# ForJadeForest/DistillCLIP

Measured on AMD Instinct MI355X. Metric: image-text pairs/sec (distill step), higher is better.
Workload: dtype bf16; 1 GPU; l_clip.yaml dual distill: ViT-B/32 CLIP teacher -> weight-shared ViT(6x768,24h,R2) + text(4x768,12h,R2) students, 224px/77tok, losses out_l1+out_cos+0.1*cos_diff, fwd+loss+bwd+AdamW; global_batch=512, batch_per_gpu=512, parallelism=dp1, gradient_exchange=none, negatives=local (reference training_step semantics), optimizer_in_step=True, teacher_residual=fp16, saved_gelu_derivative=u8 fixed point, clock_probe=True

## Files before the change

distillclip_amd/csrc/common.h:

```cpp
#pragma once
#include <hip/hip_runtime.h>
#include <stdint.h>

typedef __bf16 bf16_t;
typedef __attribute__((ext_vector_type(8))) __bf16 bf16x8;
typedef __attribute__((ext_vector_type(4))) __bf16 bf16x4;
typedef __attribute__((ext_vector_type(2))) __bf16 bf16x2;
typedef __attribute__((ext_vector_type(8))) _Float16 f16x8;
typedef __attribute__((ext_vector_type(4))) _Float16 f16x4;
typedef __attribute__((ext_vector_type(4))) short s16x4;
typedef __attribute__((ext_vector_type(4))) float f32x4;
typedef __attribute__((ext_vector_type(16))) float f32x16;
typedef __attribute__((ext_vector_type(4))) unsigned int u32x4;

#include "dclip.h"

void dclip_set_error(const char* fmt, ...);

#define DCLIP_REQUIRE(cond, ...)                 \
    do {                                          \
        if (!(cond)) {                            \
            dclip_set_error(__VA_ARGS__);         \
            return DCLIP_EINVAL;                  \
        }                                         \
    } while (0)

extern "C" int dclip_rows_pick(const void* src, void* dst, const int32_t* idx, int64_t B, int64_t row_bytes, void* stream);
extern "C" int dclip_rows_expand(const void* src, void* dst, const int32_t* idx, int64_t B, int64_t N, int64_t row_bytes, void* stream);

extern "C" int dclip_cast_bf16_pad(const float* src, void* dst, int64_t R, int64_t C, int64_t ldd, void* stream);

bool dclip_trace_open(int kind, double flops, double bytes, void* stream, int* slot, int d0 = 0, int d1 = 0, int d2 = 0, int d3 = 0);
void dclip_trace_close(int slot, void* stream);
struct TraceScope {
    int slot = -1; void* st;
    TraceScope(int kind, double flops, double bytes, void* stream, int d0 = 0, int d1 = 0, int d2 = 0, int d3 = 0) : st(stream) {
        if (!dclip_trace_open(kind, flops, bytes, stream, &slot, d0, d1, d2, d3)) slot = -1;
    }
    ~TraceScope() { if (slot >= 0) dclip_trace_close(slot, st); }
};
#define DCLIP_TRACE_GEMM_NT 0
#define DCLIP_TRACE_GEMM_TN 1
#define DCLIP_TRACE_LAYERNORM 2
#define DCLIP_TRACE_LOSS 3
#define DCLIP_TRACE_ATTN 4
#define DCLIP_TRACE_LN_BWD 5

void dclip_explain_hip_error(const char* what, int hip_error, const char* hip_text);
static inline int dclip_check_launch(const char* what) {
    hipError_t e = hipGetLastError();
    if (e != hipSuccess) {
        dclip_explain_hip_error(what, (int)e, hipGetErrorString(e));
        return DCLIP_ELAUNCH;
    }
    return DCLIP_OK;
}

static inline int grid_for(int64_t work, int per_block = 256, int cap = 2048 * 4) {
    int64_t g = (work + per_block - 1) / per_block;
    return (int)(g < 1 ? 1 : (g > cap ? cap : g));
}

static inline size_t dclip_up256(size_t x) { return (x + 255) & ~(size_t)255; }
static inline bool dclip_aligned16(const void* p) { return ((uintptr_t)p % 16) == 0; }
struct Bump {
    char* base; size_t off;
    explicit Bump(void* b) : base((char*)b), off(0) {}
    template <class T> T* take(size_t n) {
        T* p = base ? (T*)(base + off) : nullptr;
        off += dclip_up256(n * sizeof(T));
        return p;
    }
};

__device__ __forceinline__ float bf2f(bf16_t x) { return (float)x; }
__device__ __forceinline__ bf16_t f2bf(float x) { return (bf16_t)x; }

__device__ __forceinline__ float wave_sum(float v) {
#pragma unroll
    for (int o = 32; o > 0; o >>= 1) v += __shfl_xor(v, o);
    return v;
}
__device__ __forceinline__ float wave_max(float v) {
#pragma unroll
    for (int o = 32; o > 0; o >>= 1) v = fmaxf(v, __shfl_xor(v, o));
    return v;
}

__device__ __forceinline__ void wave_lds_fence() { __builtin_amdgcn_wave_barrier(); asm volatile("" ::: "memory"); __builtin_amdgcn_wave_barrier(); }

template <class T> __device__ __forceinline__ void mfma_keep_alive(const T& f) { asm volatile("" :: "v"(f)); }
template <class T> __device__ __forceinline__ void mfma_keep_alive(const T (&f)[2]) { asm volatile("" :: "v"(f[0]), "v"(f[1])); }
template <class T> __device__ __forceinline__ void mfma_keep_alive(const T (&f)[4]) { asm volatile("" :: "v"(f[0]), "v"(f[1]), "v"(f[2]), "v"(f[3])); }

__device__ __forceinline__ float quick_gelu_f(float x) { return x * __builtin_amdgcn_rcpf(1.f + __expf(-1.702f * x)); }
__device__ __forceinline__ float erf_tail(float ax_over_sqrt2, float phi) {
    const float t = __builtin_amdgcn_rcpf(fmaf(0.3275911f, ax_over_sqrt2, 1.f));
    float p = fmaf(1.061405429f, t, -1.453152027f);
    p = fmaf(p, t, 1.421413741f);
    p = fmaf(p, t, -0.284496736f);
    p = fmaf(p, t, 0.254829592f);
    return p * t * phi;
}
__device__ __forceinline__ float gelu_erf_f(float x) {
    const float phi = __expf(-0.5f * x * x);
    const float tail = erf_tail(fabsf(x) * 0.70710678118654752f, phi);
    const float cdf = x >= 0.f ? 1.f - 0.5f * tail : 0.5f * tail;
    return x * cdf;
}
__device__ __forceinline__ float dgelu_erf_f(float x) {
    const float phi = __expf(-0.5f * x * x);
    const float tail = erf_tail(fabsf(x) * 0.70710678118654752f, phi);
    const float cdf = x >= 0.f ? 1.f - 0.5f * tail : 0.5f * tail;
    return fmaf(x * phi, 0.3989422804014327f, cdf);
}

__device__ __forceinline__ void gelu_erf_both_f(float x, float& g, float& dg) {
    const float phi = __expf(-0.5f * x * x);
    const float tail = erf_tail(fabsf(x) * 0.70710678118654752f, phi);
    const float cdf = x >= 0.f ? 1.f - 0.5f * tail : 0.5f * tail;
    g = x * cdf;
    dg = fmaf(x * phi, 0.3989422804014327f, cdf);
}

#define DCLIP_DG_LO (-0.13f)
#define DCLIP_DG_STEP (1.26f / 255.f)
__device__ __forceinline__ unsigned dg_pack4(float a, float b, float c, float d) {
    const float inv = 255.f / 1.26f, off = 0.13f * (255.f / 1.26f);
    unsigned r = 0;
    r = __builtin_amdgcn_cvt_pk_u8_f32(__builtin_rintf(fmaf(a, inv, off)), 0, r);
    r = __builtin_amdgcn_cvt_pk_u8_f32(__builtin_rintf(fmaf(b, inv, off)), 1, r);
    r = __builtin_amdgcn_cvt_pk_u8_f32(__builtin_rintf(fmaf(c, inv, off)), 2, r);
    r = __builtin_amdgcn_cvt_pk_u8_f32(__builtin_rintf(fmaf(d, inv, off)), 3, r);
    return r;
}
__device__ __forceinline__ float dg_unpack(unsigned w, int byte) {
    return fmaf((float)((w >> (8 * byte)) & 0xffu), DCLIP_DG_STEP, DCLIP_DG_LO);
}

__device__ __forceinline__ bf16x8 frag_halves(s16x4 lo, s16x4 hi) {
    union { struct { s16x4 lo, hi; } s; bf16x8 v; } u;
    u.s.lo = lo; u.s.hi = hi;
    return u.v;
}

typedef __attribute__((address_space(3))) s16x4 lds_s16x4;
template <int ROWB>
__device__ __forceinline__ bf16x8 tr_frag(const char* tile, int r0, int x0, int lane) {
    const int g = lane >> 4, q = (lane >> 2) & 3, pp = lane & 3;
    const char* a0 = tile + (r0 + 8 * g + q) * ROWB + (x0 + 4 * pp) * 2;
    return frag_halves(__builtin_amdgcn_ds_read_tr16_b64_v4i16((lds_s16x4*)a0), __builtin_amdgcn_ds_read_tr16_b64_v4i16((lds_s16x4*)(a0 + 4 * ROWB)));
}

__device__ __forceinline__ int xcd_remap(int bid, int nwg) {
    const int q = nwg >> 3, r = nwg & 7, x = bid & 7;
    return (x < r ? x * (q + 1) : r * (q + 1) + (x - r) * q) + (bid >> 3);
}
```

distillclip_amd/csrc/gemm_common.h:

```cpp
#pragma once
#include <math.h>
#include <stdlib.h>
#include "common.h"
#include <type_traits>

namespace dgemm {

constexpr int BM = 128, BN = 128, BK = 64;
constexpr int SUB = 1024;
constexpr int HT = 16384;

inline unsigned long long* g_gemm_stamps = nullptr;

struct GemmNT {
    const bf16_t* A; int64_t lda;
    const bf16_t* B; int64_t ldb;
    void* C; int64_t ldc;
    int M, N, K;
    float alpha;
    const float* bias;
    const void* aux_in;
    void* aux_out;
    const void* residual; int64_t ldr;
    int row_group; const float* rowadd;
    float* colsum;
    int tiles_m, tiles_n;
    unsigned long long* stamps;
    int group_n;
    unsigned long long* clk;
};

__device__ __forceinline__ int swz(int x) { return x ^ (((x >> 9) & 1) << 5); }

typedef __attribute__((address_space(3))) void lds_void;
typedef __attribute__((address_space(1))) const void gbl_void;

struct EpiSide {
    float4 r0, r1;
    f16x8 rh;
    bf16x8 z;
    uint2 zq;
};

template <int ACT, int OUT>
__device__ __forceinline__ void epilogue_load_side(const GemmNT& p, int64_t o, int64_t orr, EpiSide& sd) {
    if (OUT == 1 && p.residual) {
        const float* rp = (const float*)p.residual + orr;
        sd.r0 = *(const float4*)rp; sd.r1 = *(const float4*)(rp + 4);
    }
    if (OUT == 2 && p.residual) sd.rh = *(const f16x8*)((const _Float16*)p.residual + orr);
    if (ACT == 3) sd.z = *(const bf16x8*)((const bf16_t*)p.aux_in + o);
    if (ACT == 4) sd.zq = *(const uint2*)((const uint8_t*)p.aux_in + o);
}

template <int ACT, int OUT, int MODE = 0, bool CSUM_ALWAYS = false>
__device__ __forceinline__ void epilogue_vec8(const GemmNT& p, float (&v)[8], int row, int col, int64_t o, int64_t orr,
                                              const float (&bias)[8], float (&csum)[8], const EpiSide& sd) {
    constexpr bool LEAN = MODE != 0;
#pragma unroll
    for (int e = 0; e < 8; ++e) v[e] = v[e] * p.alpha + bias[e];
    if (!LEAN && p.row_group > 0) {
        const float* ra = p.rowadd + (int64_t)(row % p.row_group) * p.N + col;
        const float4 a0 = *(const float4*)ra, a1 = *(const float4*)(ra + 4);
        v[0] += a0.x; v[1] += a0.y; v[2] += a0.z; v[3] += a0.w; v[4] += a1.x; v[5] += a1.y; v[6] += a1.z; v[7] += a1.w;
    }
    if (!LEAN && ACT != 5 && ACT != 6 && p.aux_out) {
        bf16x8 z;
#pragma unroll
        for (int e = 0; e < 8; ++e) z[e] = f2bf(v[e]);
        *(bf16x8*)((bf16_t*)p.aux_out + o) = z;
    }
    if (ACT == 1) {
#pragma unroll
        for (int e = 0; e < 8; ++e) v[e] = quick_gelu_f(v[e]);
    }
    if (ACT == 2) {
#pragma unroll
        for (int e = 0; e < 8; ++e) v[e] = gelu_erf_f(v[e]);
    }
    if (ACT == 3) {
        const bf16x8 z = sd.z;
#pragma unroll
        for (int e = 0; e < 8; ++e) v[e] *= dgelu_erf_f(bf2f(z[e]));
    }
    if (ACT == 4) {
        const uint2 q = sd.zq;
        v[0] *= dg_unpack(q.x, 0); v[1] *= dg_unpack(q.x, 1); v[2] *= dg_unpack(q.x, 2); v[3] *= dg_unpack(q.x, 3);
        v[4] *= dg_unpack(q.y, 0); v[5] *= dg_unpack(q.y, 1); v[6] *= dg_unpack(q.y, 2); v[7] *= dg_unpack(q.y, 3);
    }
    if (ACT == 5) {
        float dg[8];
#pragma unroll
        for (int e = 0; e < 8; ++e) {
            float g;
            gelu_erf_both_f(v[e], g, dg[e]);
            v[e] = g;
        }
        if (LEAN || p.aux_out) *(uint2*)((uint8_t*)p.aux_out + o) = uint2{dg_pack4(dg[0], dg[1], dg[2], dg[3]), dg_pack4(dg[4], dg[5], dg[6], dg[7])};
    }
    if (ACT == 6) {
        float dg[8];
#pragma unroll
        for (int e = 0; e < 8; ++e) {
            const float sg = __builtin_amdgcn_rcpf(1.f + __expf(-1.702f * v[e]));
            dg[e] = fmaf(1.702f * v[e] * sg, 1.f - sg, sg);
            v[e] *= sg;
        }
        if (LEAN || p.aux_out) *(uint2*)((uint8_t*)p.aux_out + o) = uint2{dg_pack4(dg[0], dg[1], dg[2], dg[3]), dg_pack4(dg[4], dg[5], dg[6], dg[7])};
    }
    if (MODE == 3 || (!LEAN && p.residual)) {
        if (OUT == 2) {
            const f16x8 r = sd.rh;
#pragma unroll
            for (int e = 0; e < 8; ++e) v[e] += (float)r[e];
        } else {
            float4 r0, r1;
            if (OUT == 1) { r0 = sd.r0; r1 = sd.r1; }
            else {
                const float* rp = (const float*)p.residual + orr;
                r0 = *(const float4*)rp; r1 = *(const float4*)(rp + 4);
            }
            v[0] += r0.x; v[1] += r0.y; v[2] += r0.z; v[3] += r0.w; v[4] += r1.x; v[5] += r1.y; v[6] += r1.z; v[7] += r1.w;
        }
    }
    if (OUT == 1) {
        float* cp = (float*)p.C + o;
        *(float4*)cp = float4{v[0], v[1], v[2], v[3]};
        *(float4*)(cp + 4) = float4{v[4], v[5], v[6], v[7]};
    } else if (OUT == 2) {
        f16x8 ov;
#pragma unroll
        for (int e = 0; e < 8; ++e) ov[e] = (_Float16)v[e];
        *(f16x8*)((_Float16*)p.C + o) = ov;
    } else {
        bf16x8 ov;
#pragma unroll
        for (int e = 0; e < 8; ++e) ov[e] = f2bf(v[e]);
        *(bf16x8*)((bf16_t*)p.C + o) = ov;
    }
    if (CSUM_ALWAYS || (OUT == 0 && (MODE == 2 || (MODE == 0 && p.colsum)))) {
#pragma unroll
        for (int e = 0; e < 8; ++e) csum[e] += v[e];
    }
}

#define WAIT_VMCNT(n) asm volatile("s_waitcnt vmcnt(" #n ")" ::: "memory")
#define WAIT_LGKM0() asm volatile("s_waitcnt lgkmcnt(0)" ::: "memory")

__device__ __forceinline__ void wg_stamp(unsigned long long* const& stamps, const int& tid, int k) {
    if (stamps && tid == 0) {
        if (k == 3) WAIT_VMCNT(0);
        stamps[6 * (int64_t)blockIdx.x + k] = __builtin_readcyclecounter();
        if (k == 0) stamps[6 * (int64_t)blockIdx.x + 4] = __builtin_amdgcn_s_memrealtime();
        if (k == 3) stamps[6 * (int64_t)blockIdx.x + 5] = __builtin_amdgcn_s_memrealtime();
    }
}

__device__ __forceinline__ void mfma_4x4(f32x4 (&acc)[4][4], const bf16x8 (&a)[4], const bf16x8 (&b)[4]) {
#pragma unroll
    for (int i = 0; i < 4; ++i)
#pragma unroll
        for (int j = 0; j < 4; ++j) acc[i][j] = __builtin_amdgcn_mfma_f32_16x16x32_bf16(a[i], b[j], acc[i][j], 0, 0, 0);
}

template <bool SWAP>
__device__ __forceinline__ f32x4 mfma_rc(bf16x8 rowf, bf16x8 colf, f32x4 c) {
    return SWAP ? __builtin_amdgcn_mfma_f32_16x16x32_bf16(colf, rowf, c, 0, 0, 0) : __builtin_amdgcn_mfma_f32_16x16x32_bf16(rowf, colf, c, 0, 0, 0);
}
#define PHASE_MFMA(SWAP, acc, R0, RT, af, b0, b1)                                                                         \
    do {                                                                                                                  \
        __builtin_amdgcn_s_barrier();                                                                                     \
        __builtin_amdgcn_s_setprio(1);                                                                                    \
        _Pragma("unroll") for (int kb_ = 0; kb_ < 2; ++kb_)                                                               \
            _Pragma("unroll") for (int i_ = 0; i_ < (RT); ++i_) {                                                         \
                _Pragma("unroll") for (int j_ = 0; j_ < 2; ++j_)                                                          \
                    acc[(R0) + i_][j_] = mfma_rc<SWAP>(af[i_][kb_], b0[j_][kb_], acc[(R0) + i_][j_]);                     \
                _Pragma("unroll") for (int j_ = 0; j_ < 2; ++j_)                                                          \
                    acc[(R0) + i_][2 + j_] = mfma_rc<SWAP>(af[i_][kb_], b1[j_][kb_], acc[(R0) + i_][2 + j_]);             \
            }                                                                                                             \
        __builtin_amdgcn_s_setprio(0);                                                                                    \
        __builtin_amdgcn_s_barrier();                                                                                     \
    } while (0)

template <int NI, int LD>
__device__ __forceinline__ void stage_acc(float* cs, const f32x4 (*acc)[4], int row0, int col0, int lane) {
#pragma unroll
    for (int i = 0; i < NI; ++i)
#pragma unroll
        for (int j = 0; j < 4; ++j)
#pragma unroll
            for (int r = 0; r < 4; ++r) cs[(row0 + i * 16 + (lane >> 4) * 4 + r) * LD + col0 + j * 16 + (lane & 15)] = acc[i][j][r];
}

}
```

distillclip_amd/csrc/gemm_nt.hip:

```cpp

#include "gemm_common.h"
#include <atomic>

using namespace dgemm;

namespace {

constexpr int TILE_BYTES = (BM / 16) * (BK / 32) * SUB;
constexpr int CLD = BN + 4;
constexpr int NT_LDS = (4 * TILE_BYTES > BM * CLD * 4) ? 4 * TILE_BYTES : BM * CLD * 4;


__device__ __forceinline__ void stage_operand(const bf16_t* __restrict__ G, int64_t ld, int row0, int rows_max,
                                              int k0, char* lds_tile, int wave, int lane) {
    const int L = lane * 16;
    const int X = swz(L);
    const int r = X >> 6, c = (X >> 4) & 3;
#pragma unroll
    for (int s = 0; s < 4; ++s) {
        const int sub = wave * 4 + s;
        const int rb = sub >> 1, kb = sub & 1;
        int row = row0 + rb * 16 + r;
        row = row < rows_max ? row : rows_max - 1;
        const bf16_t* src = G + (int64_t)row * ld + (k0 + kb * 32 + c * 8);
        __builtin_amdgcn_global_load_lds((gbl_void*)src, (lds_void*)(lds_tile + sub * SUB), 16, 0, 0);
    }
}

template <int ACT, int OUT>
__global__ __launch_bounds__(256) void gemm_nt_kernel(GemmNT p) {
    extern __shared__ __attribute__((aligned(16))) char smem[];
    const int tid = threadIdx.x, lane = tid & 63;
    const int wave = __builtin_amdgcn_readfirstlane(tid >> 6);
    const int wm = wave >> 1, wn = wave & 1;

    const int nwg = p.tiles_m * p.tiles_n;
    const int t = xcd_remap(blockIdx.x, nwg);
    const int tm = t / p.tiles_n, tn = t % p.tiles_n;
    const int m0 = tm * BM, n0 = tn * BN;

    char* As = smem;
    char* Bs = smem + 2 * TILE_BYTES;

    f32x4 acc[4][4];
#pragma unroll
    for (int i = 0; i < 4; ++i)
#pragma unroll
        for (int j = 0; j < 4; ++j) acc[i][j] = f32x4{0.f, 0.f, 0.f, 0.f};

    const int nk = p.K / BK;
    stage_operand(p.A, p.lda, m0, p.M, 0, As, wave, lane);
    stage_operand(p.B, p.ldb, n0, p.N, 0, Bs, wave, lane);

    const int fragoff = swz((lane & 15) * 64 + (lane >> 4) * 16);

    for (int kt = 0; kt < nk; ++kt) {
        __syncthreads();
        if (kt + 1 < nk) {
            const int nb = (kt + 1) & 1;
            stage_operand(p.A, p.lda, m0, p.M, (kt + 1) * BK, As + nb * TILE_BYTES, wave, lane);
            stage_operand(p.B, p.ldb, n0, p.N, (kt + 1) * BK, Bs + nb * TILE_BYTES, wave, lane);
        }
        const char* a_t = As + (kt & 1) * TILE_BYTES;
        const char* b_t = Bs + (kt & 1) * TILE_BYTES;
#pragma unroll
        for (int kb = 0; kb < 2; ++kb) {
            bf16x8 af[4], bfr[4];
#pragma unroll
            for (int i = 0; i < 4; ++i)
                af[i] = *(const bf16x8*)(a_t + ((wm * 4 + i) * 2 + kb) * SUB + fragoff);
#pragma unroll
            for (int j = 0; j < 4; ++j)
                bfr[j] = *(const bf16x8*)(b_t + ((wn * 4 + j) * 2 + kb) * SUB + fragoff);
            mfma_4x4(acc, af, bfr);
        }
    }

    __syncthreads();
    float* cs = (float*)smem;
    stage_acc<4, CLD>(cs, acc, wm * 64, wn * 64, lane);
    __syncthreads();
    const int cc = (tid & 15) * 8;
    const int col = n0 + cc;
    const bool col_ok = col < p.N;
    float bias[8], csum[8];
#pragma unroll
    for (int e = 0; e < 8; ++e) { bias[e] = 0.f; csum[e] = 0.f; }
    if (p.bias && col_ok) {
        const float4 b0 = *(const float4*)(p.bias + col), b1 = *(const float4*)(p.bias + col + 4);
        bias[0] = b0.x; bias[1] = b0.y; bias[2] = b0.z; bias[3] = b0.w; bias[4] = b1.x; bias[5] = b1.y; bias[6] = b1.z; bias[7] = b1.w;
    }
#pragma unroll
    for (int it = 0; it < 8; ++it) {
        const int rl = (tid >> 4) + it * 16;
        const int row = m0 + rl;
        if (row >= p.M || !col_ok) break;
        const float4 c0 = *(const float4*)(cs + rl * CLD + cc), c1 = *(const float4*)(cs + rl * CLD + cc + 4);
        float v[8] = {c0.x, c0.y, c0.z, c0.w, c1.x, c1.y, c1.z, c1.w};
        const int64_t o = (int64_t)row * p.ldc + col, orr = (int64_t)row * p.ldr + col;
        EpiSide sd;
        epilogue_load_side<ACT, OUT>(p, o, orr, sd);
        epilogue_vec8<ACT, OUT, 0, true>(p, v, row, col, o, orr, bias, csum, sd);
    }
    if (p.colsum) {
        __syncthreads();
#pragma unroll
        for (int e = 0; e < 8; ++e) cs[(tid >> 4) * CLD + cc + e] = csum[e];
        __syncthreads();
        if (tid < BN && n0 + tid < p.N) {
            float x = 0.f;
#pragma unroll
            for (int r = 0; r < 16; ++r) x += cs[r * CLD + tid];
            unsafeAtomicAdd(p.colsum + n0 + tid, x);
        }
    }
}


constexpr int nt256_lds(int mi) { return 2 * (2 * HT + 2 * (mi * 16 * BK * 2)); }

__device__ __forceinline__ void stage_half_perm(const bf16_t* __restrict__ G, int64_t ld, int row0, int rows_max, int k0,
                                                char* buf, int wave, int lane) {
    const int L = lane * 16;
    const int X = swz(L);
    const int r = X >> 6, c = (X >> 4) & 3;
    const int j = wave & 3;
    int row = row0 + (wave >> 2) * 64 + (j >> 1) * 32 + (r >> 2) * 8 + (j & 1) * 4 + (r & 3);
    row = row < rows_max ? row : rows_max - 1;
    const bf16_t* src = G + (int64_t)row * ld + k0 + c * 8;
    __builtin_amdgcn_global_load_lds((gbl_void*)src, (lds_void*)(buf + (wave * 2 + 0) * SUB), 16, 0, 0);
    __builtin_amdgcn_global_load_lds((gbl_void*)(src + 32), (lds_void*)(buf + (wave * 2 + 1) * SUB), 16, 0, 0);
}

template <int RH>
__device__ __forceinline__ void stage_rowhalf(const bf16_t* __restrict__ G, int64_t ld, int m0, int rows_max, int k0,
                                              char* abase, int hta, int dn, int wave, int lane) {
    const int L = lane * 16;
    const int X = swz(L);
    const int r = X >> 6, c = (X >> 4) & 3;
    constexpr int AROWS = RH * 32;
    {
        const int wv = RH == 3 ? wave % 6 : wave;
        const int g = wv / RH, i = wv % RH + dn * RH;
        int row = m0 + g * AROWS + i * 16 + r;
        row = row < rows_max ? row : rows_max - 1;
        const bf16_t* src = G + (int64_t)row * ld + k0 + c * 8;
        char* dst = abase + g * hta + (i * 2) * SUB;
        __builtin_amdgcn_global_load_lds((gbl_void*)src, (lds_void*)dst, 16, 0, 0);
        __builtin_amdgcn_global_load_lds((gbl_void*)(src + 32), (lds_void*)(dst + SUB), 16, 0, 0);
    }
    if (RH == 5) {
        const int e = wave & 3, rbk = 8 + (e >> 1), kb = e & 1;
        const int g = rbk / RH, i = rbk % RH + dn * RH;
        int row = m0 + g * AROWS + i * 16 + r;
        row = row < rows_max ? row : rows_max - 1;
        const bf16_t* src = G + (int64_t)row * ld + k0 + kb * 32 + c * 8;
        __builtin_amdgcn_global_load_lds((gbl_void*)src, (lds_void*)(abase + g * hta + (i * 2 + kb) * SUB), 16, 0, 0);
    }
}

__device__ __forceinline__ float row16_sum(float x) {
    auto dpp = [](float v, auto ctrl) {
        return __builtin_bit_cast(float, __builtin_amdgcn_update_dpp(0, __builtin_bit_cast(int, v), decltype(ctrl)::value, 0xf, 0xf, false));
    };
    x += dpp(x, std::integral_constant<int, 0xB1>{});
    x += dpp(x, std::integral_constant<int, 0x4E>{});
    x += dpp(x, std::integral_constant<int, 0x141>{});
    x += dpp(x, std::integral_constant<int, 0x140>{});
    return x;
}

template <int ACT, int OUT, int MI>
__global__ __launch_bounds__(512) void gemm_nt256_kernel(GemmNT p) {
    extern __shared__ __attribute__((aligned(16))) char smem[];
    constexpr int RH = MI / 2;
    constexpr int AROWS = MI * 16;
    constexpr int HTA = AROWS * BK * 2;
    constexpr int PAR = nt256_lds(MI) / 2;
    constexpr int BMT = 2 * AROWS;
    const int tid = threadIdx.x, lane = tid & 63;
    const int wave = __builtin_amdgcn_readfirstlane(tid >> 6);
    const int wr = wave >> 2, wc = wave & 3;

    const int nwg = p.tiles_m * p.tiles_n;
    const int nk = p.K / BK;
    const int nload = 4 * nk;
    int m0, n0;
    auto locate = [&](int tl) {
        const int t = xcd_remap(tl, nwg);
        int tm, tn;
        if (p.group_n >= p.tiles_n) { tm = t / p.tiles_n; tn = t % p.tiles_n; }
        else {
            const int per = p.tiles_m * p.group_n;
            const int gi = t / per, rem = t - gi * per;
            const int left = p.tiles_n - gi * p.group_n;
            const int gw = left < p.group_n ? left : p.group_n;
            tm = rem / gw; tn = gi * p.group_n + rem % gw;
        }
        m0 = tm * BMT; n0 = tn * 256;
    };
    locate(blockIdx.x);

    f32x4 acc[MI][4];

    auto issue = [&](int l) {
        const int tile = l >> 2, w = l & 3;
        char* par = smem + (tile & 1) * PAR;
        if (w < 2) stage_half_perm(p.B, p.ldb, n0 + w * 128, p.N, tile * BK, par + w * HT, wave, lane);
        else stage_rowhalf<RH>(p.A, p.lda, m0, p.M, tile * BK, par + 2 * HT, HTA, w - 2, wave, lane);
    };
    wg_stamp(p.stamps, tid, 0);
    if (p.clk && blockIdx.x == 0 && tid == 0) { p.clk[0] = __builtin_amdgcn_s_memtime(); p.clk[1] = __builtin_amdgcn_s_memrealtime(); }
#define WAIT_VM2(n8, n10) do { if (MI == 10) WAIT_VMCNT(n10); else WAIT_VMCNT(n8); } while (0)
    const int npro = nload < 7 ? nload : 7;
    for (int l = 0; l < npro; ++l) issue(l);
    const int a_off = 2 * HT + wr * HTA;
    const int b_off = (wc >> 1) * HT + (wc & 1) * 8 * SUB;
    const int fragoff = swz((lane & 15) * 64 + (lane >> 4) * 16);
#pragma unroll
    for (int i = 0; i < MI; ++i)
#pragma unroll
        for (int j = 0; j < 4; ++j) acc[i][j] = f32x4{0.f, 0.f, 0.f, 0.f};
    if (nload > 4) WAIT_VM2(8, 10); else WAIT_VMCNT(0);
    __builtin_amdgcn_s_barrier();
    wg_stamp(p.stamps, tid, 1);
    if (wr == 1) __builtin_amdgcn_s_barrier();

    bf16x8 af[RH][2], b0[2][2], b1[2][2];

    for (int kt = 0; kt < nk; ++kt) {
        const char* base = smem + (kt & 1) * PAR;
        const char* ap = base + a_off + fragoff;
        const char* bp = base + b_off + fragoff;
#pragma unroll
        for (int j = 0; j < 2; ++j)
#pragma unroll
            for (int kb = 0; kb < 2; ++kb) {
                b0[j][kb] = *(const bf16x8*)(bp + (j * 2 + kb) * SUB);
                b1[j][kb] = *(const bf16x8*)(bp + ((2 + j) * 2 + kb) * SUB);
            }
        __builtin_amdgcn_sched_barrier(0);
#pragma unroll
        for (int i = 0; i < RH; ++i)
#pragma unroll
            for (int kb = 0; kb < 2; ++kb) af[i][kb] = *(const bf16x8*)(ap + (i * 2 + kb) * SUB);
        if (kt + 1 < nk) { issue(4 * (kt + 1) + 3); WAIT_VM2(8, 10); }
        else WAIT_VMCNT(0);
        WAIT_LGKM0();
        PHASE_MFMA(true, acc, 0, RH, af, b0, b1);
#pragma unroll
        for (int i = 0; i < RH; ++i)
#pragma unroll
            for (int kb = 0; kb < 2; ++kb) af[i][kb] = *(const bf16x8*)(ap + ((RH + i) * 2 + kb) * SUB);
        if (kt + 2 < nk) { issue(4 * (kt + 2)); issue(4 * (kt + 2) + 1); issue(4 * (kt + 2) + 2); WAIT_VM2(8, 10); }
        else if (kt + 1 < nk) WAIT_VM2(2, 3);
        else WAIT_VMCNT(0);
        WAIT_LGKM0();
        PHASE_MFMA(true, acc, RH, RH, af, b0, b1);
    }
    if (wr == 0) __builtin_amdgcn_s_barrier();
    wg_stamp(p.stamps, tid, 2);
    const int g = lane >> 4, rl = lane & 15;

    const int colb = n0 + wc * 64 + g * 8;
    float bias[2][8], csum[2][8];
#pragma unroll
    for (int jp = 0; jp < 2; ++jp) {
#pragma unroll
        for (int e = 0; e < 8; ++e) { bias[jp][e] = 0.f; csum[jp][e] = 0.f; }
        const int col = colb + jp * 32;
        if (p.bias && col < p.N) {
            const float4 q0 = *(const float4*)(p.bias + col), q1 = *(const float4*)(p.bias + col + 4);
            bias[jp][0] = q0.x; bias[jp][1] = q0.y; bias[jp][2] = q0.z; bias[jp][3] = q0.w;
            bias[jp][4] = q1.x; bias[jp][5] = q1.y; bias[jp][6] = q1.z; bias[jp][7] = q1.w;
        }
    }
    constexpr bool OUT_F32 = OUT == 1;
    constexpr bool SIDE = OUT != 0 || ACT == 3 || ACT == 4;
    constexpr int NU = 2 * MI;
    constexpr int BU = !SIDE ? NU : (OUT_F32 ? ((ACT == 3 || ACT == 4) ? 4 : (MI == 8 ? 8 : (MI == 6 ? 6 : 5))) : (MI == 10 ? 10 : NU));
    static_assert(NU % BU == 0, "batch size must divide the unit count");
    EpiSide side[SIDE ? BU : 1];
    const int row0 = m0 + wr * AROWS + rl;
    const int64_t o0 = (int64_t)row0 * p.ldc + colb, r0off = (int64_t)row0 * p.ldr + colb;
    const int64_t ostep = 16 * p.ldc, rstep = 16 * p.ldr;
    const bool full = m0 + BMT <= p.M && n0 + 256 <= p.N;
    auto run_units = [&](auto mode_tag) {
        constexpr int MODE = decltype(mode_tag)::value;
#pragma unroll
        for (int ub = 0; ub < NU; ub += BU) {
            if (SIDE) {
#pragma unroll
                for (int u = ub; u < ub + BU; ++u) {
                    const int i = u >> 1, jp = u & 1;
                    if (full || (row0 + i * 16 < p.M && colb + jp * 32 < p.N))
                        epilogue_load_side<ACT, OUT>(p, o0 + i * ostep + jp * 32, r0off + i * rstep + jp * 32, side[u - ub]);
                }
            }
#pragma unroll
            for (int u = ub; u < ub + BU; ++u) {
                const int i = u >> 1, jp = u & 1;
                const int row = row0 + i * 16, col = colb + jp * 32;
                if (full || (row < p.M && col < p.N)) {
                    float v[8];
#pragma unroll
                    for (int r = 0; r < 4; ++r) { v[r] = acc[i][2 * jp][r]; v[4 + r] = acc[i][2 * jp + 1][r]; }
                    epilogue_vec8<ACT, OUT, MODE>(p, v, row, col, o0 + i * ostep + jp * 32, r0off + i * rstep + jp * 32, bias[jp], csum[jp],
                                                      side[SIDE ? u - ub : 0]);
                }
            }
        }
    };
    const bool lean = p.row_group == 0 && ((ACT == 5 || ACT == 6) ? p.aux_out != nullptr : p.aux_out == nullptr) && (OUT != 0 ? p.residual != nullptr : p.residual == nullptr);
    if constexpr (OUT != 0) {
        if (lean) run_units(std::integral_constant<int, 3>{});
        else run_units(std::integral_constant<int, 0>{});
    } else if constexpr (ACT == 3 || ACT == 4) {
        if (lean && p.colsum) run_units(std::integral_constant<int, 2>{});
        else run_units(std::integral_constant<int, 0>{});
    } else {
        if (lean && !p.colsum) run_units(std::integral_constant<int, 1>{});
        else if (lean) run_units(std::integral_constant<int, 2>{});
        else run_units(std::integral_constant<int, 0>{});
    }
    if (OUT == 0 && p.colsum) {
        float* cs = (float*)smem;
#pragma unroll
        for (int jp = 0; jp < 2; ++jp)
#pragma unroll
            for (int e = 0; e < 8; ++e) {
                const float x = row16_sum(csum[jp][e]);
                if (rl == 0) cs[wr * 256 + wc * 64 + jp * 32 + g * 8 + e] = x;
            }
        WAIT_LGKM0();
        __builtin_amdgcn_s_barrier();
        const int tc = wave * 64 + lane;
        if (tc < 256 && n0 + tc < p.N) unsafeAtomicAdd(p.colsum + n0 + tc, cs[tc] + cs[256 + tc]);
    }
    wg_stamp(p.stamps, tid, 3);
    if (p.clk && blockIdx.x == 0 && tid == 0) { p.clk[2] = __builtin_amdgcn_s_memtime(); p.clk[3] = __builtin_amdgcn_s_memrealtime(); }
}

bool use_256(const GemmNT& p) {
    static const int mode = [] { const char* e = getenv("DCLIP_GEMM256"); return e ? atoi(e) : 1; }();
    return mode != 0 && p.M >= 1024 && p.N >= 256;
}

std::atomic<unsigned long long*> g_clock_buf{nullptr};
std::atomic<long long> g_clock_cap{0};
std::atomic<long long> g_clock_count{0};
inline unsigned long long* next_clock_slot() {
    unsigned long long* buf = g_clock_buf.load(std::memory_order_acquire);
    const long long cap = g_clock_cap.load(std::memory_order_relaxed);
    if (!buf || cap <= 0) return nullptr;
    return buf + 4 * (g_clock_count.fetch_add(1, std::memory_order_relaxed) % cap);
}

int tile_height_mi(const GemmNT& p, int act, int out) {
    static const int mode320 = [] { const char* e = getenv("DCLIP_GEMM320"); return e ? atoi(e) : 1; }();
    if (!mode320) return 8;
    if (mode320 == 2) return 10;
    if (mode320 == 6) return 6;
    const int tn = (p.N + 255) / 256;
    const double nkt = (double)(p.K / BK), e8 = out == 1 ? 40000.0 : out == 2 ? 24000.0 : (act == 0 || act == 4 ? 9500.0 : 14000.0);
    auto cost = [&](int rows, double per_kt, double escale) {
        const int tmx = (p.M + rows - 1) / rows;
        return (double)((tmx * tn + 255) / 256) * (3300.0 + nkt * per_kt + escale * e8);
    };
    const double c8 = cost(256, 2750.0, 1.0), c10 = cost(320, 3200.0, 1.25), c6 = cost(192, 2150.0, 0.75);
    int mi = 8;
    if (c10 < c8) mi = 10;
    if (c6 < (mi == 10 ? c10 : c8) * 0.97) mi = 6;
    return mi;
}

int raster_group_n(const GemmNT& p) {
    const int tn = p.tiles_n, ntiles = p.tiles_m * p.tiles_n;
    const double panel = 512.0 * (double)p.K, a_bytes = 2.0 * (double)p.M * (double)p.K;
    double best = 0.0; int best_g = tn;
    for (int g = 1; g <= tn; ++g) {
        const int ngroups = (tn + g - 1) / g;
        const double b_term = (g * panel <= 2.5e6) ? 8.0 * g * panel * (ngroups > 8 ? ngroups / 8.0 : 1.0)
                                                   : (double)ntiles / 32.0 * g * panel;
        const double cost = a_bytes * ngroups + b_term;
        if (g == 1 || cost < best * 0.999) { best = cost; best_g = g; }
    }
    return best_g;
}

template <int ACT, int MI>
void launch_nt256(const GemmNT& p, int out, hipStream_t st) {
    const dim3 grid(p.tiles_m * p.tiles_n), block(512);
    constexpr size_t lds = nt256_lds(MI) + 16;
    if (out == 1) { if constexpr (ACT == 0) hipLaunchKernelGGL((gemm_nt256_kernel<0, 1, MI>), grid, block, lds, st, p); }
    else if (out == 2) { if constexpr (ACT == 0) hipLaunchKernelGGL((gemm_nt256_kernel<0, 2, MI>), grid, block, lds, st, p); }
    else hipLaunchKernelGGL((gemm_nt256_kernel<ACT, 0, MI>), grid, block, lds, st, p);
}

template <int ACT>
int launch_nt(GemmNT p, int out, hipStream_t st) {
    if constexpr (ACT != 0) { if (out == 2) { dclip_set_error("dclip_gemm_nt: f16 output needs act = DCLIP_ACT_NONE"); return DCLIP_EINVAL; } }
    if (use_256(p) && !(out != 0 && p.colsum) && (ACT == 0 || out == 0)) {
        const int mi = tile_height_mi(p, ACT, out);
        p.tiles_m = (p.M + mi * 32 - 1) / (mi * 32); p.tiles_n = (p.N + 255) / 256;
        p.clk = next_clock_slot();
        p.group_n = raster_group_n(p);
        if (mi == 10) launch_nt256<ACT, 10>(p, out, st);
        else if (mi == 6) launch_nt256<ACT, 6>(p, out, st);
        else launch_nt256<ACT, 8>(p, out, st);
        return dclip_check_launch("dclip_gemm_nt");
    }
    const int grid = p.tiles_m * p.tiles_n;
    const size_t lds = NT_LDS;
    if (out == 1) hipLaunchKernelGGL((gemm_nt_kernel<ACT, 1>), dim3(grid), dim3(256), lds, st, p);
    else if (out == 2) { if constexpr (ACT == 0) hipLaunchKernelGGL((gemm_nt_kernel<0, 2>), dim3(grid), dim3(256), lds, st, p); }
    else hipLaunchKernelGGL((gemm_nt_kernel<ACT, 0>), dim3(grid), dim3(256), lds, st, p);
    return dclip_check_launch("dclip_gemm_nt");
}

}

extern "C" int dclip_trace_gemm_stamps(void* buf) { g_gemm_stamps = (unsigned long long*)buf; return 0; }
extern "C" int64_t dclip_trace_gemm_clock(void* buf, int64_t cap) {
    const long long n = g_clock_count.exchange(0, std::memory_order_relaxed);
    g_clock_cap.store(buf ? (long long)cap : 0, std::memory_order_relaxed);
    g_clock_buf.store((unsigned long long*)buf, std::memory_order_release);
    return (int64_t)n;
}

extern "C" int dclip_gemm_nt(const void* A, int64_t lda, const void* B, int64_t ldb, void* C, int64_t ldc,
                             int64_t M, int64_t N, int64_t K, float alpha, const float* bias, int act,
                             const void* aux_in, void* aux_out, const void* residual, int64_t ldr, int out_dtype,
                             int64_t row_group, const float* rowadd, float* colsum_acc, void* stream) {
    DCLIP_REQUIRE(A && B && C, "dclip_gemm_nt: null operand");
    DCLIP_REQUIRE(M > 0 && N > 0 && K > 0, "dclip_gemm_nt: empty problem M=%ld N=%ld K=%ld", (long)M, (long)N, (long)K);
    DCLIP_REQUIRE(K % BK == 0, "dclip_gemm_nt: K=%ld must be a multiple of %d", (long)K, BK);
    DCLIP_REQUIRE(lda % 8 == 0 && ldb % 8 == 0 && ((uintptr_t)A % 16) == 0 && ((uintptr_t)B % 16) == 0,
                  "dclip_gemm_nt: operand rows must be 16-byte aligned (lda=%ld ldb=%ld)", (long)lda, (long)ldb);
    DCLIP_REQUIRE(N % 8 == 0 && ldc % 8 == 0 && ((uintptr_t)C % 16) == 0, "dclip_gemm_nt: N and ldc must be multiples of 8 and C 16-byte aligned (N=%ld ldc=%ld)", (long)N, (long)ldc);
    DCLIP_REQUIRE(out_dtype >= 0 && out_dtype <= 2, "dclip_gemm_nt: bad output dtype %d (0 bf16, 1 f32, 2 f16)", out_dtype);
    DCLIP_REQUIRE(!residual || (ldr % (out_dtype == 2 ? 8 : 4) == 0 && ((uintptr_t)residual % 16) == 0), "dclip_gemm_nt: residual rows must be 16-byte aligned");
    DCLIP_REQUIRE(act >= 0 && act <= 6, "dclip_gemm_nt: bad activation code %d", act);
    DCLIP_REQUIRE(out_dtype != 2 || act == 0, "dclip_gemm_nt: f16 output needs act = DCLIP_ACT_NONE");
    DCLIP_REQUIRE((act != DCLIP_ACT_DGELU && act != DCLIP_ACT_MULAUX) || aux_in, "dclip_gemm_nt: DGELU / MULAUX need aux_in");
    DCLIP_REQUIRE(!aux_in || ((uintptr_t)aux_in % 16) == 0, "dclip_gemm_nt: aux_in must be 16-byte aligned");
    DCLIP_REQUIRE(!aux_out || ((uintptr_t)aux_out % 16) == 0, "dclip_gemm_nt: aux_out must be 16-byte aligned");
    DCLIP_REQUIRE(row_group == 0 || rowadd, "dclip_gemm_nt: row_group needs rowadd");
    DCLIP_REQUIRE(M < (1LL << 31) && N < (1LL << 31), "dclip_gemm_nt: dimension overflow");
    GemmNT p;
    p.A = (const bf16_t*)A; p.lda = lda; p.B = (const bf16_t*)B; p.ldb = ldb; p.C = C; p.ldc = ldc;
    p.M = (int)M; p.N = (int)N; p.K = (int)K; p.alpha = alpha; p.bias = bias;
    p.aux_in = aux_in; p.aux_out = aux_out; p.residual = residual; p.ldr = ldr;
    p.row_group = (int)row_group; p.rowadd = rowadd; p.colsum = colsum_acc;
    p.tiles_m = (int)((M + BM - 1) / BM); p.tiles_n = (int)((N + BN - 1) / BN);
    p.stamps = g_gemm_stamps;
    p.group_n = 1 << 30;
    p.clk = nullptr;
    hipStream_t st = (hipStream_t)stream;
    const int out_f32 = out_dtype == 1;
    const double aux_b = (act == DCLIP_ACT_MULAUX || act == DCLIP_ACT_GELU_SAVE || act == DCLIP_ACT_QUICKGELU_SAVE) ? 1.0 : 2.0;
    TraceScope tr(DCLIP_TRACE_GEMM_NT, 2.0 * (double)M * (double)N * (double)K,
                  2.0 * ((double)M * K + (double)N * K) + ((out_f32 ? 4.0 : 2.0) + (residual ? (out_dtype == 2 ? 2.0 : 4.0) : 0.0) + (aux_in ? aux_b : 0.0) + (aux_out ? aux_b : 0.0)) * (double)M * N,
                  stream, (int)M, (int)N, (int)K,
                  act + 8 * (out_f32 != 0) + 16 * (residual != nullptr) + 32 * (colsum_acc != nullptr) + 64 * (out_dtype == 2));
    switch (act) {
        case 0: return launch_nt<0>(p, out_dtype, st);
        case 1: return launch_nt<1>(p, out_dtype, st);
        case 2: return launch_nt<2>(p, out_dtype, st);
        case 3: return launch_nt<3>(p, out_dtype, st);
        case 4: return launch_nt<4>(p, out_dtype, st);
        case 5: return launch_nt<5>(p, out_dtype, st);
        default: return launch_nt<6>(p, out_dtype, st);
    }
}
```

Before: 18520 pairs/s.

## Prefetch GELU-derivative aux tile into LDS during last K step; pack GELU math

For the ACT==4 GEMM epilogue (multiply by the saved u8 GELU derivative), the u8 aux tile is now fetched by asynchronous global-to-LDS loads issued during the final K iteration. The epilogue then reads it from LDS instead of issuing global loads after the main loop. Separately, the erf-GELU forward-with-derivative epilogue (ACT==5) and dg_pack4 are rewritten on float2 vectors so the compiler can use packed FP32 ops, with exp2 and copysign replacing branches. The change adds wait-count tuning, an extra LDS parity dependency and moves the colsum scratch to the other parity buffer, which raises the risk of LDS hazards.

Result: no change. 18650 pairs/s (median of 6 runs) (+0.7%).

```diff
diff --git a/distillclip_amd/csrc/common.h b/distillclip_amd/csrc/common.h
--- a/distillclip_amd/csrc/common.h
+++ b/distillclip_amd/csrc/common.h
@@ -115,25 +115,38 @@
     return fmaf(x * phi, 0.3989422804014327f, cdf);
 }
 
-__device__ __forceinline__ void gelu_erf_both_f(float x, float& g, float& dg) {
-    const float phi = __expf(-0.5f * x * x);
-    const float tail = erf_tail(fabsf(x) * 0.70710678118654752f, phi);
-    const float cdf = x >= 0.f ? 1.f - 0.5f * tail : 0.5f * tail;
+typedef __attribute__((ext_vector_type(2))) float f32x2;
+__device__ __forceinline__ f32x2 f32x2_of(float v) { return f32x2{v, v}; }
+__device__ __forceinline__ void gelu_erf_both_f2(f32x2 x, f32x2& g, f32x2& dg) {
+    const f32x2 e = ((-0.5f * x) * x) * 1.44269504088896341f;
+    const f32x2 phi = f32x2{__builtin_amdgcn_exp2f(e.x), __builtin_amdgcn_exp2f(e.y)};
+    const f32x2 a = x * 0.70710678118654752f;
+    const f32x2 t = f32x2{__builtin_amdgcn_rcpf(fmaf(0.3275911f, __builtin_fabsf(a.x), 1.f)),
+                          __builtin_amdgcn_rcpf(fmaf(0.3275911f, __builtin_fabsf(a.y), 1.f))};
+    f32x2 p = __builtin_elementwise_fma(f32x2_of(1.061405429f), t, f32x2_of(-1.453152027f));
+    p = __builtin_elementwise_fma(p, t, f32x2_of(1.421413741f));
+    p = __builtin_elementwise_fma(p, t, f32x2_of(-0.284496736f));
+    p = __builtin_elementwise_fma(p, t, f32x2_of(0.254829592f));
+    const f32x2 tail = (p * t) * phi;
+    const f32x2 m = f32x2{__builtin_copysignf(0.5f, x.x), __builtin_copysignf(0.5f, x.y)};
+    const f32x2 cdf = __builtin_elementwise_fma(tail, -m, m + 0.5f);
     g = x * cdf;
-    dg = fmaf(x * phi, 0.3989422804014327f, cdf);
+    dg = __builtin_elementwise_fma(x * phi, f32x2_of(0.3989422804014327f), cdf);
 }
 
 #define DCLIP_DG_LO (-0.13f)
 #define DCLIP_DG_STEP (1.26f / 255.f)
-__device__ __forceinline__ unsigned dg_pack4(float a, float b, float c, float d) {
-    const float inv = 255.f / 1.26f, off = 0.13f * (255.f / 1.26f);
+__device__ __forceinline__ unsigned dg_pack4(f32x2 ab, f32x2 cd) {
+    const f32x2 inv = f32x2_of(255.f / 1.26f), off = f32x2_of(0.13f * (255.f / 1.26f));
+    const f32x2 q0 = __builtin_elementwise_fma(ab, inv, off), q1 = __builtin_elementwise_fma(cd, inv, off);
     unsigned r = 0;
-    r = __builtin_amdgcn_cvt_pk_u8_f32(__builtin_rintf(fmaf(a, inv, off)), 0, r);
-    r = __builtin_amdgcn_cvt_pk_u8_f32(__builtin_rintf(fmaf(b, inv, off)), 1, r);
-    r = __builtin_amdgcn_cvt_pk_u8_f32(__builtin_rintf(fmaf(c, inv, off)), 2, r);
-    r = __builtin_amdgcn_cvt_pk_u8_f32(__builtin_rintf(fmaf(d, inv, off)), 3, r);
+    r = __builtin_amdgcn_cvt_pk_u8_f32(q0.x, 0, r);
+    r = __builtin_amdgcn_cvt_pk_u8_f32(q0.y, 1, r);
+    r = __builtin_amdgcn_cvt_pk_u8_f32(q1.x, 2, r);
+    r = __builtin_amdgcn_cvt_pk_u8_f32(q1.y, 3, r);
     return r;
 }
+__device__ __forceinline__ unsigned dg_pack4(float a, float b, float c, float d) { return dg_pack4(f32x2{a, b}, f32x2{c, d}); }
 __device__ __forceinline__ float dg_unpack(unsigned w, int byte) {
     return fmaf((float)((w >> (8 * byte)) & 0xffu), DCLIP_DG_STEP, DCLIP_DG_LO);
 }
diff --git a/distillclip_amd/csrc/gemm_common.h b/distillclip_amd/csrc/gemm_common.h
--- a/distillclip_amd/csrc/gemm_common.h
+++ b/distillclip_amd/csrc/gemm_common.h
@@ -89,14 +89,14 @@
         v[4] *= dg_unpack(q.y, 0); v[5] *= dg_unpack(q.y, 1); v[6] *= dg_unpack(q.y, 2); v[7] *= dg_unpack(q.y, 3);
     }
     if (ACT == 5) {
-        float dg[8];
+        f32x2 dg[4];
 #pragma unroll
-        for (int e = 0; e < 8; ++e) {
-            float g;
-            gelu_erf_both_f(v[e], g, dg[e]);
-            v[e] = g;
+        for (int e = 0; e < 4; ++e) {
+            f32x2 g;
+            gelu_erf_both_f2(f32x2{v[2 * e], v[2 * e + 1]}, g, dg[e]);
+            v[2 * e] = g.x; v[2 * e + 1] = g.y;
         }
-        if (LEAN || p.aux_out) *(uint2*)((uint8_t*)p.aux_out + o) = uint2{dg_pack4(dg[0], dg[1], dg[2], dg[3]), dg_pack4(dg[4], dg[5], dg[6], dg[7])};
+        if (LEAN || p.aux_out) *(uint2*)((uint8_t*)p.aux_out + o) = uint2{dg_pack4(dg[0], dg[1]), dg_pack4(dg[2], dg[3])};
     }
     if (ACT == 6) {
         float dg[8];
diff --git a/distillclip_amd/csrc/gemm_nt.hip b/distillclip_amd/csrc/gemm_nt.hip
--- a/distillclip_amd/csrc/gemm_nt.hip
+++ b/distillclip_amd/csrc/gemm_nt.hip
@@ -200,6 +200,24 @@
         m0 = tm * BMT; n0 = tn * 256;
     };
     locate(blockIdx.x);
+    const bool full = m0 + BMT <= p.M && n0 + 256 <= p.N;
+
+    constexpr bool AUXL = ACT == 4 && OUT == 0;
+    const bool aux_dma = AUXL && full && p.ldc < (1ll << 27);
+    constexpr int NAUXT = MI == 10 ? 9 : MI;
+    static_assert(8 * NAUXT * SUB <= PAR, "the aux rows of the 8 waves must fit one parity");
+    char* const aux_lds = smem + (nk & 1) * PAR + wave * (NAUXT * SUB);
+    auto issue_aux = [&]() {
+        unsigned ones = ~0u;
+        asm volatile("" : "+s"(ones));
+        const int l = __builtin_amdgcn_mbcnt_hi(ones, __builtin_amdgcn_mbcnt_lo(ones, 0));
+        const uint32_t loff = (uint32_t)(l >> 2) * (uint32_t)p.ldc + (uint32_t)(l & 3) * 16u;
+        const uint8_t* base = (const uint8_t*)p.aux_in + (int64_t)(m0 + wr * AROWS) * p.ldc + (n0 + wc * 64);
+#pragma unroll
+        for (int i = 0; i < NAUXT; ++i)
+            __builtin_amdgcn_global_load_lds((gbl_void*)(base + (int64_t)i * 16 * p.ldc + loff), (lds_void*)(aux_lds + i * SUB), 16, 0, 0);
+    };
+#define WAIT_VM_AUX() do { if (MI == 10) WAIT_VMCNT(9); else if (MI == 8) WAIT_VMCNT(8); else WAIT_VMCNT(6); } while (0)
 
     f32x4 acc[MI][4];
 
@@ -229,7 +247,9 @@
     bf16x8 af[RH][2], b0[2][2], b1[2][2];
 
     for (int kt = 0; kt < nk; ++kt) {
-        const char* base = smem + (kt & 1) * PAR;
+        int par = kt & 1;
+        if (AUXL) asm volatile("s_nop 1" : "+s"(par));
+        const char* base = smem + par * PAR;
         const char* ap = base + a_off + fragoff;
         const char* bp = base + b_off + fragoff;
 #pragma unroll
@@ -245,6 +265,7 @@
 #pragma unroll
             for (int kb = 0; kb < 2; ++kb) af[i][kb] = *(const bf16x8*)(ap + (i * 2 + kb) * SUB);
         if (kt + 1 < nk) { issue(4 * (kt + 1) + 3); WAIT_VM2(8, 10); }
+        else if (AUXL && aux_dma) { issue_aux(); WAIT_VM_AUX(); }
         else WAIT_VMCNT(0);
         WAIT_LGKM0();
         PHASE_MFMA(true, acc, 0, RH, af, b0, b1);
@@ -254,6 +275,7 @@
             for (int kb = 0; kb < 2; ++kb) af[i][kb] = *(const bf16x8*)(ap + ((RH + i) * 2 + kb) * SUB);
         if (kt + 2 < nk) { issue(4 * (kt + 2)); issue(4 * (kt + 2) + 1); issue(4 * (kt + 2) + 2); WAIT_VM2(8, 10); }
         else if (kt + 1 < nk) WAIT_VM2(2, 3);
+        else if (AUXL && aux_dma) WAIT_VM_AUX();
         else WAIT_VMCNT(0);
         WAIT_LGKM0();
         PHASE_MFMA(true, acc, RH, RH, af, b0, b1);
@@ -284,7 +306,6 @@
     const int row0 = m0 + wr * AROWS + rl;
     const int64_t o0 = (int64_t)row0 * p.ldc + colb, r0off = (int64_t)row0 * p.ldr + colb;
     const int64_t ostep = 16 * p.ldc, rstep = 16 * p.ldr;
-    const bool full = m0 + BMT <= p.M && n0 + 256 <= p.N;
     auto run_units = [&](auto mode_tag) {
         constexpr int MODE = decltype(mode_tag)::value;
 #pragma unroll
@@ -311,11 +332,41 @@
             }
         }
     };
+    auto run_units_lds = [&](auto mode_tag) {
+        constexpr int MODE = decltype(mode_tag)::value;
+        constexpr int NREST = NU - 2 * NAUXT;
+        EpiSide rest[NREST > 0 ? NREST : 1];
+#pragma unroll
+        for (int u = 2 * NAUXT; u < NU; ++u)
+            epilogue_load_side<ACT, OUT>(p, o0 + (u >> 1) * ostep + (u & 1) * 32, r0off + (u >> 1) * rstep + (u & 1) * 32, rest[u - 2 * NAUXT]);
+        WAIT_VMCNT(0);
+        const char* zl = aux_lds + rl * 64 + g * 8;
+        uint2 zq_next = *(const uint2*)zl;
+#pragma unroll
+        for (int u = 0; u < NU; ++u) {
+            const int i = u >> 1, jp = u & 1;
+            EpiSide sd;
+            if (i < NAUXT) sd.zq = zq_next;
+            else sd = rest[u >= 2 * NAUXT ? u - 2 * NAUXT : 0];
+            if (u + 1 < 2 * NAUXT) zq_next = *(const uint2*)(zl + ((u + 1) >> 1) * SUB + ((u + 1) & 1) * 32);
+            float v[8];
+#pragma unroll
+            for (int r = 0; r < 4; ++r) { v[r] = acc[i][2 * jp][r]; v[4 + r] = acc[i][2 * jp + 1][r]; }
+            epilogue_vec8<ACT, OUT, MODE>(p, v, row0 + i * 16, colb + jp * 32, o0 + i * ostep + jp * 32, r0off + i * rstep + jp * 32, bias[jp], csum[jp], sd);
+            __builtin_amdgcn_sched_barrier(0);
+        }
+    };
     const bool lean = p.row_group == 0 && ((ACT == 5 || ACT == 6) ? p.aux_out != nullptr : p.aux_out == nullptr) && (OUT != 0 ? p.residual != nullptr : p.residual == nullptr);
     if constexpr (OUT != 0) {
         if (lean) run_units(std::integral_constant<int, 3>{});
         else run_units(std::integral_constant<int, 0>{});
-    } else if constexpr (ACT == 3 || ACT == 4) {
+    } else if constexpr (AUXL) {
+        if (aux_dma) {
+            if (lean && p.colsum) run_units_lds(std::integral_constant<int, 2>{});
+            else run_units_lds(std::integral_constant<int, 0>{});
+        } else if (lean && p.colsum) run_units(std::integral_constant<int, 2>{});
+        else run_units(std::integral_constant<int, 0>{});
+    } else if constexpr (ACT == 3) {
         if (lean && p.colsum) run_units(std::integral_constant<int, 2>{});
         else run_units(std::integral_constant<int, 0>{});
     } else {
@@ -323,8 +374,14 @@
         else if (lean) run_units(std::integral_constant<int, 2>{});
         else run_units(std::integral_constant<int, 0>{});
     }
+#ifdef DCLIP_STAMP_TAIL
+    if (p.stamps && tid == 0) {
+        WAIT_VMCNT(0);
+        p.stamps[6 * (int64_t)blockIdx.x + 2] = __builtin_readcyclecounter();
+    }
+#endif
     if (OUT == 0 && p.colsum) {
-        float* cs = (float*)smem;
+        float* cs = (float*)(smem + ((nk + 1) & 1) * PAR);
 #pragma unroll
         for (int jp = 0; jp < 2; ++jp)
 #pragma unroll
```
